# soldasim/BOSS.jl

Measured on AMD Instinct MI355X. Metric: gp_posterior_updates_per_sec (+ acq_evals_per_sec), N=4096 d=8 fp64, higher is better.
Workload: dtype f64; 1 GPU; d=8 synthetic blackbox, GaussianProcess(Matern52) surrogate, N=4096 fp64 posterior update + ExpectedImprovement over 8192 candidates per GPU (BASELINE.json configs[1]+[2]); N=4096, d=8, M_per_gpu=8192, kernel=matern52, parallelism=single GPU: no exchange

## Files before the change

### boss.jl_amd/csrc/chain.hpp

```cpp
#pragma once
#include "potrf.hpp"

namespace boss {

#ifdef BOSS_CHAIN_TRACE
__device__ unsigned long long g_ctrace[64 * 16];
#define CTRACE(step, slot) do { if ((threadIdx.x & 63) == 0) g_ctrace[((step) & 63) * 16 + (slot)] = __builtin_amdgcn_s_memrealtime(); } while (0)
#define CTRACE_MIN(step, slot) do { if (threadIdx.x == 0) atomicMin(&g_ctrace[((step) & 63) * 16 + (slot)], (unsigned long long)__builtin_amdgcn_s_memrealtime()); } while (0)
#define CTRACE_MAX(step, slot) do { if (threadIdx.x == 0) atomicMax(&g_ctrace[((step) & 63) * 16 + (slot)], (unsigned long long)__builtin_amdgcn_s_memrealtime()); } while (0)
#else
#define CTRACE(step, slot) do { } while (0)
#define CTRACE_MIN(step, slot) do { } while (0)
#define CTRACE_MAX(step, slot) do { } while (0)
#endif

#define CHAIN_CUT_VGPRS() asm volatile("" ::: "memory", "v0","v1","v2","v3","v4","v5","v6","v7","v8","v9","v10","v11","v12","v13","v14","v15","v16","v17","v18","v19","v20","v21","v22","v23","v24","v25","v26","v27","v28","v29","v30","v31","v32","v33","v34","v35","v36","v37","v38","v39","v40","v41","v42","v43","v44","v45","v46","v47","v48","v49","v50","v51","v52","v53","v54","v55","v56","v57","v58","v59","v60","v61","v62","v63","v64","v65","v66","v67","v68","v69","v70","v71","v72","v73","v74","v75","v76","v77","v78","v79","v80","v81","v82","v83","v84","v85","v86","v87","v88","v89","v90","v91","v92","v93","v94","v95","v96","v97","v98","v99","v100","v101","v102","v103","v104","v105","v106","v107","v108","v109","v110","v111")
constexpr int STRIPS_LDS_BYTES = 90 * 1024;
constexpr int CHAIN_CTRL = DIAG_TILES * 256 + DIAG_STAGE;
constexpr int CHAIN_LDS_BYTES = (CHAIN_CTRL + 2) * 8;


__device__ const unsigned char chain_tile_tab[16][3] = {
    {7, 0, 3}, {7, 3, 3}, {7, 6, 2}, {6, 0, 3}, {6, 3, 2}, {6, 5, 2}, {5, 0, 3}, {5, 3, 3},
    {4, 0, 3}, {4, 3, 2}, {3, 0, 2}, {3, 2, 2}, {2, 0, 3}, {1, 0, 2}, {0, 0, 1}, {0, 0, 0}};
__device__ __forceinline__ void chain_follow_phase(double* __restrict__ A, int ld, int b, int* __restrict__ info,
                                                             unsigned long long* __restrict__ sig, unsigned long long base, int wave_s,
                                                             unsigned budget) {
    extern __shared__ double smem[];
    int lane = (int)__builtin_amdgcn_mbcnt_hi(~0u, __builtin_amdgcn_mbcnt_lo(~0u, 0u));
    asm volatile("" : "+v"(lane));
    const int wave = wave_s, tid = wave * 64 + lane;
    const int r16 = lane & 15, q = lane >> 4;
    const int ti = chain_tile_tab[wave][0], tj0 = chain_tile_tab[wave][1], nt = chain_tile_tab[wave][2];
    constexpr int U = 3;
    const double* Ab = A + (size_t)b * BLK * ((size_t)ld + 1) + (size_t)q * ld + ti * 16 + r16;
    v4d cr[U];
#pragma unroll
    for (int u = 0; u < U; ++u) {
        const int tj = min(tj0 + u, ti);
#pragma unroll
        for (int i = 0; i < 4; ++i) cr[u][i] = ld_sc1(Ab + (size_t)(tj * 16 + 4 * i) * ld);
    }
    const unsigned long long pbase = base + 8ull * (b - 1);
    const double* Pl = A + (size_t)b * BLK + (size_t)(b - 1) * BLK * ld + (size_t)q * ld + r16;
    volatile lds_int_t* seenw = (volatile lds_int_t*)(unsigned)(unsigned long long)(smem + CHAIN_CTRL) + 1;
    auto poll_strips = [&]() {
        const unsigned long long v = lane < 8 ? ld_word(sig + SIGW_PROG + SIGW_PROG_STRIDE * lane) : ~0ull;
        const unsigned long long cnt = (v > pbase) ? v - pbase : 0ull;
        int mn = cnt > 8ull ? 8 : (int)cnt;
        mn = min(mn, __shfl_xor(mn, 1));
        mn = min(mn, __shfl_xor(mn, 2));
        mn = min(mn, __shfl_xor(mn, 4));
        return __builtin_amdgcn_readfirstlane(mn);
    };
    int seen = 0, jb = 0;
    bool dead = false;
    if (wave == 15) {
        if (lane == 0) CTRACE(b, 1);
        const PollTimer tm(budget);
        for (int it = 0; it < POLL_CAP && seen < 8; ++it) {
            const int mn = poll_strips();
            asm volatile("" ::: "memory");
            if (mn > seen) {
                seen = mn;
                if (lane == 0) *seenw = seen;
            }
            if (tm.check(it, info)) break;
            __builtin_amdgcn_s_sleep(1);
        }
        if (seen < 8) {
            if (lane == 0) {
                st_info(info, INT_MIN);
                note_giveup(4, b);
                *seenw = 99;
            }
        }
        if (lane == 0) CTRACE(b, 2);
        jb = 8;
    }
#pragma unroll 1
    while (jb < 8) {
        if (!dead && seen <= jb) {
            bool got = false;
            for (int it = 0; it < POLL_CAP_LDS; ++it) {
                const int v = *seenw;
                if (v > jb) {
                    seen = v;
                    got = v <= 8;
                    break;
                }
                __builtin_amdgcn_s_sleep(1);
            }
            if (!got) dead = true;
        }
        const bool two = (dead || seen >= jb + 2) && jb + 2 <= 8;
        const double* Pj = Pl + (size_t)(jb * 16) * ld;
        double bf[2][4], af[2][U][4];
#pragma unroll
        for (int s4 = 0; s4 < 4; ++s4) {
            bf[0][s4] = ld_sc1(Pj + (size_t)(4 * s4) * ld + ti * 16);
#pragma unroll
            for (int u = 0; u < U; ++u) af[0][u][s4] = ld_sc1(Pj + (size_t)(4 * s4) * ld + min(tj0 + u, ti) * 16);
        }
        if (two) {
#pragma unroll
            for (int s4 = 0; s4 < 4; ++s4) {
                bf[1][s4] = ld_sc1(Pj + (size_t)(16 + 4 * s4) * ld + ti * 16);
#pragma unroll
                for (int u = 0; u < U; ++u) af[1][u][s4] = ld_sc1(Pj + (size_t)(16 + 4 * s4) * ld + min(tj0 + u, ti) * 16);
            }
        }
#ifdef BOSS_CHAIN_TRACE
        if (wave == 0 && jb + (two ? 2 : 1) == 8) {
            asm volatile("s_waitcnt vmcnt(0)" ::: "memory");
            CTRACE(b, 11);
        }
#endif
#pragma unroll
        for (int s4 = 0; s4 < 4; ++s4)
#pragma unroll
            for (int u = 0; u < U; ++u) cr[u] = mfma_f64(-af[0][u][s4], bf[0][s4], cr[u]);
        if (two) {
#pragma unroll
            for (int s4 = 0; s4 < 4; ++s4)
#pragma unroll
                for (int u = 0; u < U; ++u) cr[u] = mfma_f64(-af[1][u][s4], bf[1][s4], cr[u]);
        }
        jb += two ? 2 : 1;
        if (!dead) {
            const int v = *seenw;
            if (v > seen && v <= 8) seen = v;
        }
    }
#pragma unroll
    for (int u = 0; u < U; ++u) {
        if (u < nt) {
            double* ct = smem + (ti * (ti + 1) / 2 + tj0 + u) * 256 + q * 16 + r16;
#pragma unroll
            for (int i = 0; i < 4; ++i) ct[64 * i] = cr[u][i];
        }
    }
    if (wave == 0) CTRACE(b, 12);
}

__device__ __forceinline__ void chain_factor_phase(double* __restrict__ Ab, int ld, double* __restrict__ inv16b, int col0,
                                                             unsigned long long* __restrict__ pubword, unsigned long long seq0,
                                                             int* __restrict__ info, int wave_s) {
    extern __shared__ double smem[];
    int fail = -1;
    int tid = wave_s * 64 + (int)__builtin_amdgcn_mbcnt_hi(~0u, __builtin_amdgcn_mbcnt_lo(~0u, 0u));
    asm volatile("" : "+v"(tid));
    diag_block_factor<false, false, true>(smem, Ab, ld, inv16b, col0, 8, fail, nullptr, pubword, seq0, info, tid + 0x10000);
}

__device__ __forceinline__ int chain_lane_opaque() {
    int lane = (int)__builtin_amdgcn_mbcnt_hi(~0u, __builtin_amdgcn_mbcnt_lo(~0u, 0u));
    asm volatile("" : "+v"(lane));
    return lane;
}

__global__ __launch_bounds__(DIAG_THREADS) void potrf_chain_kernel(double* __restrict__ A, int ld, int nblk,
                                                                   double* __restrict__ inv16, int* __restrict__ info,
                                                                   unsigned long long* __restrict__ sig, unsigned long long base,
                                                                   unsigned long long cbase, unsigned budget) {
    extern __shared__ double smem[];
    const int wave = __builtin_amdgcn_readfirstlane((int)threadIdx.x >> 6);
    volatile lds_int_t* ctrl = (volatile lds_int_t*)(unsigned)(unsigned long long)(smem + CHAIN_CTRL);
    asm volatile("" ::: "v127");
    if (threadIdx.x == 0) __hip_atomic_fetch_add(as_global(sig + SIGW_UP), 1ull, __ATOMIC_RELAXED, __HIP_MEMORY_SCOPE_AGENT);
    for (int b = blockIdx.x; b < nblk; b += gridDim.x) {
        double* Ab = A + (size_t)b * BLK * ((size_t)ld + 1);
        if (wave == 0) {
            const bool ok = b < 2 ? poll_ge(sig + SIGW_WDONE, base + 1, info, budget) : poll_ge(sig + SIGW_CRIT, cbase + 8ull * (b - 1), info, budget);
            if (chain_lane_opaque() == 0) {
                *ctrl = ok ? 1 : -1;
                ctrl[1] = 0;
            }
        }
        __syncthreads();
        if (*ctrl < 0) return;
        if (wave == 0) CTRACE(b, 0);
        __builtin_amdgcn_fence(__ATOMIC_ACQUIRE, "agent");
        if (b == 0) {
            const int lane = chain_lane_opaque();
            for (int tl = wave; tl < DIAG_TILES; tl += DIAG_THREADS / 64) {
                int ti = 0;
                while ((ti + 1) * (ti + 2) / 2 <= tl) ++ti;
                const int tj = tl - ti * (ti + 1) / 2;
#pragma unroll
                for (int h = 0; h < 2; ++h) {
                    const int e = lane + 64 * h, c = e >> 3, rp = e & 7;
                    *reinterpret_cast<v2d*>(smem + tl * 256 + c * 16 + 2 * rp) =
                        *reinterpret_cast<const v2d*>(Ab + (size_t)(tj * 16 + c) * ld + ti * 16 + 2 * rp);
                }
            }
        } else {
            CHAIN_CUT_VGPRS();
            chain_follow_phase(A, ld, b, info, sig, base, wave, budget);
        }
        CHAIN_CUT_VGPRS();
        __syncthreads();
        if (wave == 0) CTRACE(b, 3);
        chain_factor_phase(Ab, ld, inv16 + (size_t)b * (8 * 256), b * BLK, sig + SIGW_PANEL, base + 8ull * b, info, wave);
        CHAIN_CUT_VGPRS();
        if (wave == 15) CTRACE(b, 4);
        __syncthreads();
    }
}

template <bool CRIT>
__device__ __forceinline__ void follow_strip(double* __restrict__ A, int ld, int k, const double* __restrict__ inv16base,
                                             double* __restrict__ Brow, unsigned long long* __restrict__ prog,
                                             unsigned long long* __restrict__ sig, unsigned long long base, int* __restrict__ info,
                                             v4d (&xs)[TRSM_NA][64], int& ready, int& drained, int& avail, unsigned budget) {
    constexpr bool crit = CRIT;
    const int lane = threadIdx.x & 63;
    const int wave = __builtin_amdgcn_readfirstlane(threadIdx.x >> 6);
    const double* Lkk = A + (size_t)k * BLK * ((size_t)ld + 1);
    const double* inv16k = inv16base + (size_t)k * (8 * 256);
    const unsigned long long pb = base + 8ull * k;
    auto bload = [&](const double* p) { return crit ? ld_sc1(p) : *p; };
    auto panels_out = [&](unsigned long long v) { return v > pb ? (v - pb > 8ull ? 8 : (int)(v - pb)) : 0; };
    if (threadIdx.x == 0) {
        *(volatile lds_int_t*)&ready = 0;
        *(volatile lds_int_t*)&drained = 0;
        *(volatile lds_int_t*)&avail = panels_out(ld_word(sig + SIGW_PANEL));
    }
    __syncthreads();
    auto lval = [&](int jb, int m, int s) { return ld_sc1(Lkk + (size_t)(m * 16 + 4 * s + (lane >> 4)) * ld + jb * 16 + (lane & 15)); };
    auto ival = [&](int jb, int s) { return ld_sc1(inv16k + jb * 256 + (4 * s + (lane >> 4)) * 16 + (lane & 15)); };
    bool dead = false;
    auto ival_poll = [&](int jb, double (&iv)[4]) {
        const PollTimer tm(budget);
        for (int it = 0; it < POLL_CAP; ++it) {
            bool miss = false;
#pragma unroll
            for (int s = 0; s < 4; ++s) {
                iv[s] = ival(jb, s);
                miss |= __double_as_longlong(iv[s]) == -1ll;
            }
            if (!__any(miss)) return;
            if (dead) return;
            if (tm.check(it, info)) break;
            __builtin_amdgcn_s_sleep(1);
        }
        if (!dead && lane == 0) {
            st_info(info, INT_MIN);
            note_giveup(8, k);
        }
        dead = true;
        if (wave == 0 && lane == 0) *(volatile lds_int_t*)&avail = 99;
    };
    auto store_tile = [&](int jb, const v4d& t) {
#pragma unroll
        for (int i = 0; i < 4; ++i) {
            double* dst = Brow + (lane & 15) + (size_t)(jb * 16 + (lane >> 4) + 4 * i) * ld;
            if (crit) st_sc1(dst, t[i]);
            else *dst = t[i];
        }
    };
    int seen = *(volatile lds_int_t*)&avail;
    auto await = [&](int jb) {
        if (dead || seen > jb) return;
        if (wave == 0) {
            const PollTimer tm(budget);
            for (int i = 0; i < POLL_CAP; ++i) {
                seen = panels_out(ld_word(sig + SIGW_PANEL));
                if (seen > jb) {
                    asm volatile("" ::: "memory");
                    if (lane == 0) *(volatile lds_int_t*)&avail = seen;
                    return;
                }
                if (tm.check(i, info)) break;
                __builtin_amdgcn_s_sleep(crit ? 1 : 8);
            }
            dead = true;
            if (lane == 0) {
                st_info(info, INT_MIN);
                note_giveup(crit ? 5 : 6, k);
                *(volatile lds_int_t*)&avail = 99;
            }
        } else {
            for (int i = 0; i < POLL_CAP_LDS; ++i) {
                seen = *(volatile lds_int_t*)&avail;
                if (seen > jb) {
                    asm volatile("" ::: "memory");
                    if (seen > 8) dead = true;
                    return;
                }
                __builtin_amdgcn_s_sleep(2);
            }
            dead = true;
        }
    };
    const bool late = seen >= 8;
#ifdef BOSS_CHAIN_TRACE
    if (crit && blockIdx.x == 0 && threadIdx.x == 0) g_ctrace[(k & 63) * 16 + 7] = late ? 1 : 0;
    if (crit && blockIdx.x == 0 && threadIdx.x == 0) g_ctrace[(k & 63) * 16 + 8] = __builtin_amdgcn_s_memrealtime();
#endif
    if (wave == 0) {
        v4d acc[TRSM_NA];
#pragma unroll
        for (int jb = 0; jb < TRSM_NA; ++jb)
#pragma unroll
            for (int i = 0; i < 4; ++i) acc[jb][i] = bload(Brow + (lane & 15) + (size_t)(jb * 16 + (lane >> 4) + 4 * i) * ld);
        if (late) {
            double lv[TRSM_NA][TRSM_NA][4], iv[TRSM_NA][4];
#pragma unroll
            for (int jb = 0; jb < TRSM_NA; ++jb) {
#pragma unroll
                for (int s = 0; s < 4; ++s) iv[jb][s] = ival(jb, s);
#pragma unroll
                for (int m = 0; m < jb; ++m)
#pragma unroll
                    for (int s = 0; s < 4; ++s) lv[jb][m][s] = lval(jb, m, s);
            }
#pragma unroll
            for (int jb = 0; jb < TRSM_NA; ++jb) {
#pragma unroll
                for (int m = 0; m < jb; ++m)
#pragma unroll
                    for (int s = 0; s < 4; ++s) acc[jb] = mfma_f64(-lv[jb][m][s], acc[m][s], acc[jb]);
                v4d nw = {0.0, 0.0, 0.0, 0.0};
#pragma unroll
                for (int s = 0; s < 4; ++s) nw = mfma_f64(iv[jb][s], acc[jb][s], nw);
                acc[jb] = nw;
                xs[jb][lane] = nw;
                asm volatile("s_waitcnt lgkmcnt(0)" ::: "memory");
                if (lane == 0) *(volatile lds_int_t*)&ready = jb + 1;
            }
#pragma unroll
            for (int jb = 0; jb < TRSM_NA; ++jb) store_tile(jb, acc[jb]);
            if (crit) {
                drain_stores();
                if (lane == 0) raise_word(prog, pb + TRSM_NA);
            }
        } else {
#pragma unroll
            for (int jb = 0; jb < TRSM_NA; ++jb) {
                double iv[4], lv[TRSM_NA][4];
                if (crit) {
                    ival_poll(jb, iv);
                } else {
                    await(jb);
#pragma unroll
                    for (int s = 0; s < 4; ++s) iv[s] = ival(jb, s);
#pragma unroll
                    for (int j = jb + 1; j < TRSM_NA; ++j)
#pragma unroll
                        for (int s = 0; s < 4; ++s) lv[j][s] = lval(j, jb, s);
                }
                v4d nw = {0.0, 0.0, 0.0, 0.0};
#pragma unroll
                for (int s = 0; s < 4; ++s) nw = mfma_f64(iv[s], acc[jb][s], nw);
                acc[jb] = nw;
                xs[jb][lane] = nw;
                asm volatile("s_waitcnt lgkmcnt(0)" ::: "memory");
                if (lane == 0) *(volatile lds_int_t*)&ready = jb + 1;
                store_tile(jb, nw);
                if (crit) {
                    drain_stores();
                    if (lane == 0) raise_word(prog, pb + jb + 1);
                    await(jb);
#pragma unroll
                    for (int j = jb + 1; j < TRSM_NA; ++j)
#pragma unroll
                        for (int s = 0; s < 4; ++s) lv[j][s] = lval(j, jb, s);
                }
#pragma unroll
                for (int j = jb + 1; j < TRSM_NA; ++j)
#pragma unroll
                    for (int s = 0; s < 4; ++s) acc[j] = mfma_f64(-lv[j][s], nw[s], acc[j]);
            }
        }
        if (crit) {
            asm volatile("s_waitcnt vmcnt(0) lgkmcnt(0)" ::: "memory");
            if (lane == 0) *(volatile lds_int_t*)&drained = 1;
        }
#pragma unroll 1
        for (int jb = TRSM_NA; jb < 8; ++jb) await(jb);
    } else {
        constexpr int NB = 8 - TRSM_NA;
        v4d acc[NB];
#pragma unroll
        for (int j = 0; j < NB; ++j)
#pragma unroll
            for (int i = 0; i < 4; ++i) acc[j][i] = bload(Brow + (lane & 15) + (size_t)((TRSM_NA + j) * 16 + (lane >> 4) + 4 * i) * ld);
        auto hand_off = [&](int m) {
            while (*(volatile lds_int_t*)&ready <= m) __builtin_amdgcn_s_sleep(1);
            asm volatile("" ::: "memory");
            return xs[m][lane];
        };
        auto publish = [&](int upto) {
            if (!crit) return;
            drain_stores();
            while (*(volatile lds_int_t*)&drained == 0) __builtin_amdgcn_s_sleep(1);
            if (lane == 0) raise_word(prog, pb + upto);
        };
        if (late) {
            double lu[TRSM_NA][NB][4], lo[NB][NB][4], iv[NB][4];
#pragma unroll
            for (int m = 0; m < TRSM_NA; ++m)
#pragma unroll
                for (int j = 0; j < NB; ++j)
#pragma unroll
                    for (int s = 0; s < 4; ++s) lu[m][j][s] = lval(TRSM_NA + j, m, s);
#pragma unroll
            for (int j = 0; j < NB; ++j) {
#pragma unroll
                for (int s = 0; s < 4; ++s) iv[j][s] = ival(TRSM_NA + j, s);
#pragma unroll
                for (int m = 0; m < j; ++m)
#pragma unroll
                    for (int s = 0; s < 4; ++s) lo[j][m][s] = lval(TRSM_NA + j, TRSM_NA + m, s);
            }
#pragma unroll
            for (int m = 0; m < TRSM_NA; ++m) {
                const v4d x = hand_off(m);
#pragma unroll
                for (int s = 0; s < 4; ++s)
#pragma unroll
                    for (int j = 0; j < NB; ++j) acc[j] = mfma_f64(-lu[m][j][s], x[s], acc[j]);
            }
#pragma unroll
            for (int j = 0; j < NB; ++j) {
#pragma unroll
                for (int m = 0; m < j; ++m)
#pragma unroll
                    for (int s = 0; s < 4; ++s) acc[j] = mfma_f64(-lo[j][m][s], acc[m][s], acc[j]);
                v4d nw = {0.0, 0.0, 0.0, 0.0};
#pragma unroll
                for (int s = 0; s < 4; ++s) nw = mfma_f64(iv[j][s], acc[j][s], nw);
                acc[j] = nw;
            }
#pragma unroll
            for (int j = 0; j < NB; ++j) store_tile(TRSM_NA + j, acc[j]);
            publish(8);
        } else {
#pragma unroll
            for (int m = 0; m < TRSM_NA; ++m) {
                await(m);
                double lu[NB][4];
#pragma unroll
                for (int j = 0; j < NB; ++j)
#pragma unroll
                    for (int s = 0; s < 4; ++s) lu[j][s] = lval(TRSM_NA + j, m, s);
                const v4d x = hand_off(m);
#pragma unroll
                for (int s = 0; s < 4; ++s)
#pragma unroll
                    for (int j = 0; j < NB; ++j) acc[j] = mfma_f64(-lu[j][s], x[s], acc[j]);
            }
#pragma unroll
            for (int j = 0; j < NB; ++j) {
                double iv[4], lo[NB][4];
                if (crit) {
                    ival_poll(TRSM_NA + j, iv);
                } else {
                    await(TRSM_NA + j);
#pragma unroll
                    for (int s = 0; s < 4; ++s) iv[s] = ival(TRSM_NA + j, s);
#pragma unroll
                    for (int j2 = j + 1; j2 < NB; ++j2)
#pragma unroll
                        for (int s = 0; s < 4; ++s) lo[j2][s] = lval(TRSM_NA + j2, TRSM_NA + j, s);
                }
                v4d nw = {0.0, 0.0, 0.0, 0.0};
#pragma unroll
                for (int s = 0; s < 4; ++s) nw = mfma_f64(iv[s], acc[j][s], nw);
                acc[j] = nw;
                store_tile(TRSM_NA + j, nw);
                if (crit) {
                    publish(TRSM_NA + j + 1);
                    if (j + 1 < NB) {
                        await(TRSM_NA + j);
#pragma unroll
                        for (int j2 = j + 1; j2 < NB; ++j2)
#pragma unroll
                            for (int s = 0; s < 4; ++s) lo[j2][s] = lval(TRSM_NA + j2, TRSM_NA + j, s);
                    }
                }
#pragma unroll
                for (int j2 = j + 1; j2 < NB; ++j2)
#pragma unroll
                    for (int s = 0; s < 4; ++s) acc[j2] = mfma_f64(-lo[j2][s], nw[s], acc[j2]);
                if (!crit) publish(TRSM_NA + j + 1);
            }
        }
    }
}

__global__ __launch_bounds__(TRSM_THREADS) void potrf_follow_kernel(double* __restrict__ A, int ld, int k,
                                                                    const double* __restrict__ inv16base, int row0, int wait_rows,
                                                                    unsigned long long* __restrict__ sig, unsigned long long base,
                                                                    unsigned long long gateval, int* __restrict__ info, unsigned budget) {
    if (blockIdx.x == 0 && threadIdx.x == 0) {
        raise_word(sig + SIGW_WDONE, base + k + 1);
        if (gateval) raise_word(sig + SIGW_GATE, gateval);
    }
    __builtin_amdgcn_s_setprio(3);
    CTRACE_MIN(k, 5);
    __shared__ v4d xs[TRSM_NA][64];
// ... 70 lines not shown
```

### boss.jl_amd/csrc/potrf.hpp

```cpp
#pragma once
#include "gemm_f64.hpp"

namespace boss {

#ifdef BOSS_CHAIN_TRACE
__device__ unsigned long long g_cutrace[64 * 4];
__device__ unsigned long long g_ptrace[64 * 32];
#define PTRACE(col0, jb, slot) do { if ((threadIdx.x & 63) == 0) g_ptrace[(((col0) / BLK) & 63) * 32 + (slot) * 8 + (jb)] = __builtin_amdgcn_s_memrealtime(); } while (0)
#else
#define PTRACE(col0, jb, slot) do { } while (0)
#endif

__device__ __forceinline__ void lds_barrier() { asm volatile("s_waitcnt lgkmcnt(0)\n\ts_barrier" ::: "memory"); }


__device__ __forceinline__ void chol16_unscaled(v4d& S, v4d& E, double (&ipsel)[4], int lane, int col0, int& fail) {
    const int r16 = lane & 15, q = lane >> 4;
#pragma unroll
    for (int i = 0; i < 4; ++i) E[i] = (r16 == q + 4 * i) ? 1.0 : 0.0;
    bool bad = false;
    int badcol = 0;
#pragma unroll
    for (int t = 0; t < 4; ++t) {
        ipsel[t] = 1.0;
        double p = readlane_f64(S[t], 4 * t);
#pragma unroll
        for (int j = 0; j < 4; ++j) {
            double dn = 0.0, ln = 0.0, lS = 0.0, lE = 0.0, lc = 0.0;
            if (j < 3) {
                dn = readlane_f64(S[t], 16 * (j + 1) + 4 * t + j + 1);
                ln = readlane_f64(S[t], 16 * j + 4 * t + j + 1);
                lS = __shfl(S[t], 16 * j + r16);
                lE = __shfl(E[t], 16 * j + r16);
                lc = __shfl(S[t], 16 * j + 4 * t + q);
            }
            if (!(p > 0.0) && !bad) {
                bad = true;
                badcol = 4 * t + j;
            }
            const double ip = rcp_refined(p);
            ipsel[t] = (q == j) ? ip : ipsel[t];
            if (j < 3) {
                p = __builtin_fma(-ln, ln * ip, dn);
                const double lcm = (q > j) ? lc : 0.0;
                const double m = lcm * ip;
                S[t] = __builtin_fma(-lS, m, S[t]);
                E[t] = __builtin_fma(-lE, m, E[t]);
            }
        }
        if (t < 3) {
            const double am = (r16 > 4 * t + 3) ? -S[t] * ipsel[t] : 0.0;
            const double bS = S[t], bE = E[t];
            S = mfma_f64(am, bS, S);
            E = mfma_f64(am, bE, E);
        }
    }
    if (bad && fail < 0) fail = col0 + badcol;
}

__device__ __forceinline__ int lp_index(int R, int C) { return ((R * 4 + (C & 3)) * 4) + (C >> 2); }

typedef __attribute__((address_space(3))) int lds_int_t;
typedef __attribute__((address_space(1))) unsigned long long gmem_u64;
typedef __attribute__((address_space(1))) int gmem_i32;
__device__ __forceinline__ gmem_u64* as_global(const void* p) { return (gmem_u64*)(unsigned long long)p; }
__device__ __forceinline__ void st_sc1(double* p, double v) {
    __hip_atomic_store(as_global(p), (unsigned long long)__double_as_longlong(v), __ATOMIC_RELAXED, __HIP_MEMORY_SCOPE_AGENT);
}
__device__ __forceinline__ double ld_sc1(const double* p) {
    return __longlong_as_double((long long)__hip_atomic_load(as_global(p), __ATOMIC_RELAXED, __HIP_MEMORY_SCOPE_AGENT));
}
__device__ __forceinline__ unsigned long long ld_word(const unsigned long long* w) {
    return __hip_atomic_load(as_global(w), __ATOMIC_RELAXED, __HIP_MEMORY_SCOPE_AGENT);
}
__device__ __forceinline__ int ld_info(const int* p) {
    return __hip_atomic_load((gmem_i32*)(unsigned long long)p, __ATOMIC_RELAXED, __HIP_MEMORY_SCOPE_AGENT);
}
__device__ __forceinline__ void st_info(int* p, int v) {
    __hip_atomic_store((gmem_i32*)(unsigned long long)p, v, __ATOMIC_RELAXED, __HIP_MEMORY_SCOPE_AGENT);
}
__device__ __forceinline__ int ld_info_fresh(const int* p) {
    int r;
    const int zero = 0;
    asm volatile("global_atomic_or %0, %1, %2, off sc0\n\ts_waitcnt vmcnt(0)" : "=&v"(r) : "v"((gmem_i32*)(unsigned long long)p), "v"(zero) : "memory");
    return r;
}
__device__ __forceinline__ void st_sc1_x4(double* p, v2d v) {
    asm volatile("global_store_dwordx4 %0, %1, off sc1\n\ts_nop 1" ::"v"(as_global(p)), "v"(v) : "memory");
}
__device__ __forceinline__ void drain_stores() { asm volatile("s_waitcnt vmcnt(0)" ::: "memory"); }
__device__ __forceinline__ void raise_word(unsigned long long* w, unsigned long long v) {
    __hip_atomic_store(as_global(w), v, __ATOMIC_RELAXED, __HIP_MEMORY_SCOPE_AGENT);
}
constexpr int SIGW_GATE = 0, SIGW_BULK = 3, SIGW_PANEL = 16, SIGW_WDONE = 32, SIGW_CRIT = 48, SIGW_NEAR = 8, SIGW_PROG = 64, SIGW_PROG_STRIDE = 16,
              SIGW_UP = SIGW_PROG + 8 * SIGW_PROG_STRIDE,
              SIGW_DBG = SIGW_UP + 16,
              SIG_WORDS = SIGW_DBG + 16;
__device__ int g_giveup = 0;
#ifdef BOSS_DEBUG_WATCH_BUILD
__device__ unsigned long long* g_dbg = nullptr;
#endif
__device__ __forceinline__ void note_giveup(int code, int detail) {
    atomicCAS(&g_giveup, 0, code * 1000 + (detail & 511));
#ifdef BOSS_DEBUG_WATCH_BUILD
    unsigned long long* d = g_dbg;
    if (d) {
        atomicCAS(d + SIGW_DBG, 0ull, (unsigned long long)(code * 1000 + (detail & 511)));
        atomicAdd(d + SIGW_DBG + 1, 1ull);
        d[SIGW_DBG + 2] = (unsigned long long)(code * 1000 + (detail & 511));
    }
#endif
}
constexpr int POLL_CAP = 1 << 26;
constexpr int POLL_CAP_LDS = 1 << 22;
struct PollTimer {
    unsigned long long t0;
    unsigned budget;
    __device__ __forceinline__ explicit PollTimer(unsigned b) : t0(__builtin_amdgcn_s_memrealtime()), budget(b) {}
    __device__ __forceinline__ bool expired() const { return __builtin_amdgcn_s_memrealtime() - t0 > (unsigned long long)budget; }
    __device__ __forceinline__ int check(int i, const int* info) const {
        if ((i & 63) != 63) return 0;
        if (ld_info(info) == INT_MIN) return 2;
        if ((i & 1023) == 1023) {
            const int v = ld_info_fresh(info);
#ifdef BOSS_DEBUG_WATCH_BUILD
            if (v == INT_MIN && g_dbg && (threadIdx.x & 63) == 0) atomicAdd(g_dbg + SIGW_DBG + 4, 1ull);
#endif
            if (v == INT_MIN) return 2;
        }
        const bool out = expired();
#ifdef BOSS_DEBUG_WATCH_BUILD
        if (out && g_dbg && (threadIdx.x & 63) == 0) atomicAdd(g_dbg + SIGW_DBG + 5, 1ull);
#endif
        return out ? 1 : 0;
    }
};
__device__ __forceinline__ bool poll_ge(const unsigned long long* w, unsigned long long v, int* info, unsigned budget) {
    const PollTimer tm(budget);
    for (int i = 0; i < POLL_CAP; ++i) {
        if (ld_word(w) >= v) {
            asm volatile("" ::: "memory");
            return true;
        }
        const int st = tm.check(i, info);
        if (st == 2) return false;
        if (st == 1) break;
        __builtin_amdgcn_s_sleep(1);
    }
    if ((threadIdx.x & 63) == 0) {
        st_info(info, INT_MIN);
        note_giveup(1, (int)(v & 511));
    }
    return false;
}

constexpr int DIAG_THREADS = 1024;
constexpr int DIAG_TILES = 36;
constexpr int DIAG_STAGE = 2 * 256 + 2;
constexpr int DIAG_LDS_BYTES = (DIAG_TILES * 256 + DIAG_STAGE) * 8;
__device__ __forceinline__ int dtile(int i, int j) { return (i * (i + 1) / 2 + j) * 256; }
__device__ __forceinline__ double inv16_entry(double v) {
    const long long b = __double_as_longlong(v);
    return (b & 0x7fffffffffffffffll) > 0x7ff0000000000000ll ? __longlong_as_double(0x7ff8000000000000ll) : v;
}

template <bool KEEP = false, bool TILE0_GLOBAL = false, bool PUB = false>
__device__ __forceinline__ void diag_block_factor(double* __restrict__ smem, double* __restrict__ A, int ld,
                                                  double* __restrict__ inv16, int col0, int nsub, int& fail,
                                                  double* __restrict__ Is = nullptr, unsigned long long* pubword = nullptr,
                                                  unsigned long long pubseq0 = 0, int* info = nullptr, int tidtok = 0) {
    double* D = smem;
    double* Es = smem + DIAG_TILES * 256;
    double* Ss = Es + 256;
    volatile lds_int_t* xread = (volatile lds_int_t*)(unsigned)(unsigned long long)(Ss + 256);
    const int tid = tidtok >= 0x10000 ? tidtok - 0x10000 : (int)threadIdx.x + tidtok, lane = tid & 63;
    const int wave = __builtin_amdgcn_readfirstlane(tid >> 6);
    const int r16 = lane & 15, q = lane >> 4;
    constexpr int NW = DIAG_THREADS / 64;
    if (tid == 0) *xread = 0;
    v4d S = {0.0, 0.0, 0.0, 0.0};
    int osym[4], oel[4];
#pragma unroll
    for (int i = 0; i < 4; ++i) {
        const int c = q + 4 * i;
        osym[i] = (r16 >= c) ? (c * 16 + r16) : (r16 * 16 + c);
        oel[i] = c * 16 + r16;
    }
    int oe[4], od[4];
#pragma unroll
    for (int i = 0; i < 4; ++i) {
        oe[i] = lp_index(4 * i + q, r16);
        od[i] = lp_index(q + 4 * i, q + 4 * i);
    }
    const int olp = (r16 * 4 + q) * 4;
    if (wave == 0) {
#pragma unroll
        for (int i = 0; i < 4; ++i) {
            if constexpr (TILE0_GLOBAL) {
                const int c = q + 4 * i;
                S[i] = (r16 >= c) ? A[(size_t)c * ld + r16] : A[(size_t)r16 * ld + c];
            } else {
                S[i] = D[osym[i]];
            }
        }
    }
    for (int jb = 0; jb < nsub; ++jb) {
        const int t = nsub - 1 - jb;
        double ipsel[4];
        if (wave == 0) {
            v4d E;
            if constexpr (PUB) PTRACE(col0, jb, 0);
            chol16_unscaled(S, E, ipsel, lane, col0 + jb * 16, fail);
            if constexpr (PUB) PTRACE(col0, jb, 1);
            *reinterpret_cast<v4d*>(Es + olp) = E;
            *reinterpret_cast<v4d*>(Ss + olp) = S;
            if constexpr (PUB) {
                if (fail >= 0) {
                    if (lane == 0 && ld_info(info) == 0) st_info(info, fail + 1);
                    drain_stores();
                }
            }
        } else if (jb > 0 && (wave & 3) != 0 && !(PUB && wave == 15)) {
            const int jp = jb - 1, tp = nsub - 1 - jp;
            const int T = tp * (tp + 1) / 2;
            constexpr int U = 2;
            constexpr int NUPD = NW - NW / 4 - (PUB ? 1 : 0);
            const int uw = wave - 1 - (wave >> 2);
            for (int q0 = 1 + uw; q0 < T; q0 += U * NUPD) {
                int ti[U], tj[U];
                bool ok[U];
                v4d cr[U];
                double* ct[U];
#pragma unroll
                for (int u = 0; u < U; ++u) {
                    const int qq = q0 + NUPD * u;
                    ok[u] = qq < T;
                    int a = 0;
                    while ((a + 1) * (a + 2) / 2 <= qq) ++a;
                    const int b = qq - a * (a + 1) / 2;
                    ti[u] = ok[u] ? jp + 1 + a : jp + 2;
                    tj[u] = ok[u] ? jp + 1 + b : jp + 2;
                    ct[u] = D + dtile(ti[u], tj[u]);
#pragma unroll
                    for (int i = 0; i < 4; ++i) cr[u][i] = ct[u][oel[i]];
                }
#pragma unroll
                for (int s4 = 0; s4 < 4; ++s4) {
                    double af[U], bf[U];
#pragma unroll
                    for (int u = 0; u < U; ++u) {
                        af[u] = D[dtile(tj[u], jp) + oel[s4]];
                        bf[u] = D[dtile(ti[u], jp) + oel[s4]];
                    }
#pragma unroll
                    for (int u = 0; u < U; ++u) cr[u] = mfma_f64(-af[u], bf[u], cr[u]);
                }
#pragma unroll
                for (int u = 0; u < U; ++u) {
                    if (ok[u]) {
#pragma unroll
                        for (int i = 0; i < 4; ++i) ct[u][oel[i]] = cr[u][i];
                    }
                }
            }
        }
        lds_barrier();
        if (wave == 15) {
            const v4d Sv = *reinterpret_cast<const v4d*>(Ss + olp), Ev = *reinterpret_cast<const v4d*>(Es + olp);
            double* At = A + (size_t)(jb * 16) * ((size_t)ld + 1);
#pragma unroll
            for (int i = 0; i < 4; ++i) {
                const double rs = rsqrt_refined(Ss[od[i]]);
                const int c = q + 4 * i;
                if constexpr (PUB) {
                    if (r16 >= c) st_sc1(At + (size_t)c * ld + r16, Sv[i] * rs);
                    st_sc1(inv16 + jb * 256 + r16 * 16 + c, inv16_entry(Ev[i] * rs));
                } else {
                    if (r16 >= c) At[(size_t)c * ld + r16] = Sv[i] * rs;
                    inv16[jb * 256 + r16 * 16 + c] = inv16_entry(Ev[i] * rs);
                }
                if constexpr (KEEP) {
                    D[dtile(jb, jb) + oel[i]] = (r16 >= c) ? Sv[i] * rs : 0.0;
                    Is[jb * 256 + r16 * 16 + c] = Ev[i] * rs;
                }
            }
            if constexpr (PUB) {
                if (t == 0) {
                    drain_stores();
                    if (lane == 0) raise_word(pubword, pubseq0 + jb + 1);
                }
            }
        }
        if (t == 0) break;
        if (wave == 0) {
            const int tn = jb + 1;
            v4d P = {0.0, 0.0, 0.0, 0.0};
            const double* Dx = D + dtile(tn, jb);
            double aop[4], bop[4];
#pragma unroll
            for (int s4 = 0; s4 < 4; ++s4) {
                aop[s4] = Es[oe[s4]];
                bop[s4] = Dx[oel[s4]];
            }
            const double* Dn = D + dtile(tn, tn);
#pragma unroll
            for (int i = 0; i < 4; ++i) S[i] = Dn[osym[i]];
#pragma unroll
            for (int s4 = 0; s4 < 4; ++s4) P = mfma_f64(aop[s4], bop[s4], P);
            if (lane == 0) *xread = jb + 1;
#pragma unroll
            for (int s4 = 0; s4 < 4; ++s4) S = mfma_f64(-P[s4] * ipsel[s4], P[s4], S);
        } else if ((wave & 3) != 0 && wave - (wave >> 2) <= t) {
            const int wi = wave - (wave >> 2);
            const int tr = jb + wi;
            v4d P = {0.0, 0.0, 0.0, 0.0};
            double rs[4];
            double* Xt = D + dtile(tr, jb);
#pragma unroll
            for (int i = 0; i < 4; ++i) rs[i] = Ss[od[i]];
#pragma unroll
            for (int s4 = 0; s4 < 4; ++s4) {
                const double aop = Es[oe[s4]];
                const double bop = Xt[oel[s4]];
                P = mfma_f64(aop, bop, P);
            }
            double pv[4];
#pragma unroll
            for (int i = 0; i < 4; ++i) pv[i] = P[i] * rsqrt_refined(rs[i]);
            if (wi == 1) {
                while (*xread < jb + 1) __builtin_amdgcn_s_sleep(1);
            }
#pragma unroll
            for (int i = 0; i < 4; ++i) Xt[oel[i]] = pv[i];
        }
        lds_barrier();
        if constexpr (PUB) {
            if (wave == 15) {
                for (int tr = jb + 1; tr < nsub; ++tr) {
                    const double* src = D + dtile(tr, jb);
#pragma unroll
                    for (int h = 0; h < 2; ++h) {
                        const int e = lane + 64 * h, c = e >> 3, rp = e & 7;
                        st_sc1_x4(A + (size_t)(jb * 16 + c) * ld + tr * 16 + 2 * rp, *reinterpret_cast<const v2d*>(src + c * 16 + 2 * rp));
                    }
                }
                PTRACE(col0, jb, 2);
                drain_stores();
                PTRACE(col0, jb, 3);
                if (lane == 0) raise_word(pubword, pubseq0 + jb + 1);
            }
        }
        if constexpr (TILE0_GLOBAL) {
            if (wave == 12) {
                for (int tr = jb + 1; tr < nsub; ++tr) {
                    const double* src = D + dtile(tr, jb);
#pragma unroll
                    for (int h = 0; h < 2; ++h) {
                        const int e = lane + 64 * h, c = e >> 3, rp = e & 7;
                        *reinterpret_cast<v2d*>(A + (size_t)(jb * 16 + c) * ld + tr * 16 + 2 * rp) =
                            *reinterpret_cast<const v2d*>(src + c * 16 + 2 * rp);
                    }
                }
            }
        }
    }
}

__global__ __launch_bounds__(64) void potrf_gate_kernel(unsigned long long* __restrict__ sig, unsigned long long v,
                                                        int* __restrict__ info, unsigned budget) {
    if (threadIdx.x != 0) return;
    const PollTimer tm(budget);
    for (int i = 0; i < POLL_CAP; ++i) {
        if (__hip_atomic_load(sig, __ATOMIC_RELAXED, __HIP_MEMORY_SCOPE_AGENT) >= v) return;
        if ((i & 63) == 63 && tm.expired()) break;
        __builtin_amdgcn_s_sleep(16);
    }
    info[0] = INT_MIN;
    note_giveup(3, (int)(v & 511));
}

__global__ __launch_bounds__(64) void potrf_publish_kernel(unsigned long long* __restrict__ word, unsigned long long v) {
    if (threadIdx.x == 0) __hip_atomic_store(word, v, __ATOMIC_RELAXED, __HIP_MEMORY_SCOPE_AGENT);
}
__device__ __forceinline__ void wait_word(unsigned long long* w, unsigned long long v, int* info, unsigned budget) {
    if (!w) return;
    __shared__ int waited_s;
    if (threadIdx.x == 0) {
        bool ok = false, waited = false;
        const PollTimer tm(budget);
        for (int i = 0; i < POLL_CAP; ++i) {
            if (ld_word(w) >= v) {
                ok = true;
                break;
            }
            waited = true;
            if (tm.check(i, info)) break;
            __builtin_amdgcn_s_sleep(16);
        }
        if (!ok) {
            st_info(info, INT_MIN);
            note_giveup(2, (int)(v & 511));
        }
        *(volatile lds_int_t*)&waited_s = waited ? 1 : 0;
    }
    __syncthreads();
    if (*(volatile lds_int_t*)&waited_s) __builtin_amdgcn_fence(__ATOMIC_ACQUIRE, "agent");
}

__global__ __launch_bounds__(DIAG_THREADS) void potrf_diag_kernel(double* __restrict__ Abase, int ld, size_t bstride,
                                                                  int k, double* __restrict__ inv16base,
                                                                  size_t inv16_bstride, int* __restrict__ info,
                                                                  unsigned long long* sig, unsigned long long sigval) {
    extern __shared__ double smem[];
    const int tid = threadIdx.x;
    if (sig && tid == 0 && blockIdx.z == 0) __hip_atomic_store(sig, sigval, __ATOMIC_RELAXED, __HIP_MEMORY_SCOPE_AGENT);
    double* A = Abase + (size_t)blockIdx.z * bstride + (size_t)k * BLK * ((size_t)ld + 1);
    double* inv16 = inv16base + (size_t)blockIdx.z * inv16_bstride + (size_t)k * (8 * 256);
    const int lane = tid & 63, wv = tid >> 6;
    if (wv != 0) {
        for (int tl = wv; tl < DIAG_TILES; tl += DIAG_THREADS / 64 - 1) {
            int ti = 0;
            while ((ti + 1) * (ti + 2) / 2 <= tl) ++ti;
            const int tj = tl - ti * (ti + 1) / 2;
#pragma unroll
            for (int h = 0; h < 2; ++h) {
                const int e = lane + 64 * h, c = e >> 3, rp = e & 7;
                *reinterpret_cast<v2d*>(smem + tl * 256 + c * 16 + 2 * rp) =
                    *reinterpret_cast<const v2d*>(A + (size_t)(tj * 16 + c) * ld + ti * 16 + 2 * rp);
            }
        }
    }
    int fail = -1;
    diag_block_factor<false, true>(smem, A, ld, inv16, k * BLK, 8, fail);
    if (tid == 0 && fail >= 0) {
        if (info[blockIdx.z] == 0) info[blockIdx.z] = fail + 1;
    }
}

constexpr int SMALL_MAX_N = BLK, SMALL_MAX_D = 32;
struct SmallFitPar {
    int d, N, Np, ld, kern;
    double amp2, sig2;
    double invlam[SMALL_MAX_D];
};
constexpr int SMALL_LDS_DOUBLES = DIAG_TILES * 256 + DIAG_STAGE + 2 + 8 * 256 + SMALL_MAX_D * SMALL_MAX_N + 2 * SMALL_MAX_N + 8 + SMALL_MAX_D;
constexpr int SMALL_LDS_BYTES = SMALL_LDS_DOUBLES * 8;

__device__ __forceinline__ void small_fit_body(double* __restrict__ smem, int d, int N, int Np, int ld, int kern, double amp2,
                                               double sig2, const double* __restrict__ ilam, const double* __restrict__ Xraw,
                                               double* __restrict__ Xsc, const double* __restrict__ y,
                                               const double* __restrict__ mean, double* __restrict__ A,
                                               double* __restrict__ inv16, double* __restrict__ par_dev,
                                               double* __restrict__ scal, int* __restrict__ info,
                                               double* __restrict__ host_res, unsigned long long res_seq = 0) {
    double* Is = smem + DIAG_TILES * 256 + DIAG_STAGE + 2;
    double* xs = Is + 8 * 256;
    double* rhs = xs + SMALL_MAX_D * SMALL_MAX_N;
    double* red = rhs + 2 * SMALL_MAX_N;
    const int tid = threadIdx.x, lane = tid & 63, wv = tid >> 6;
    const int nsub = (N + 15) / 16;
    __syncthreads();
    if (par_dev) {
        if (tid < d) par_dev[tid] = ilam[tid];
        if (tid == 0) {
            par_dev[d] = amp2;
            par_dev[d + 1] = sig2;
        }
    }
    for (int idx = tid; idx < d * Np; idx += DIAG_THREADS) {
        const int k = idx / Np, j = idx - k * Np;
        const double v = Xraw[idx] * ilam[k];
        Xsc[idx] = v;
        if (j < SMALL_MAX_N) xs[k * SMALL_MAX_N + j] = v;
    }
    if (tid < SMALL_MAX_N) rhs[tid] = (tid < N) ? y[tid] - (mean ? mean[tid] : 0.0) : 0.0;
    __syncthreads();
    const int ntl = nsub * (nsub + 1) / 2;
    for (int idx = tid; idx < ntl * 256; idx += DIAG_THREADS) {
        const int tl = idx >> 8, e = idx & 255;
        int ti = 0;
        while ((ti + 1) * (ti + 2) / 2 <= tl) ++ti;
        const int tj = tl - ti * (ti + 1) / 2;
        const int r = e & 15, c = e >> 4, i = ti * 16 + r, j = tj * 16 + c;
        double v = 0.0;
        if (i >= j) {
            if (i < N && j < N) {
                double r2 = 0.0;
                for (int k = 0; k < d; ++k) {
                    const double diff = xs[k * SMALL_MAX_N + i] - xs[k * SMALL_MAX_N + j];
                    r2 = __builtin_fma(diff, diff, r2);
                }
                v = amp2 * kappa_r2(kern, r2) + ((i == j) ? sig2 : 0.0);
            } else {
                v = (i == j) ? 1.0 : 0.0;
            }
        }
        smem[tl * 256 + c * 16 + r] = v;
    }
    __syncthreads();
    int fail = -1;
    diag_block_factor<true>(smem, A, ld, inv16, 0, nsub, fail, Is);
    __syncthreads();
    if (wv == 0) {
        const int r16 = lane & 15, q = lane >> 4;
        double acc0 = 0.0, acc1 = 0.0;
        for (int jb = 0; jb < nsub; ++jb) {
            const int row0 = 16 * jb;
            if (lane >= (row0 & 63) && lane < (row0 & 63) + 16) rhs[row0 + (lane - (row0 & 63))] -= (row0 < 64) ? acc0 : acc1;
            double zs = 0.0;
#pragma unroll
            for (int i = 0; i < 4; ++i) {
                const int c = q + 4 * i;
                zs = __builtin_fma(Is[jb * 256 + c * 16 + r16], rhs[row0 + c], zs);
            }
            zs += __shfl_xor(zs, 16);
            zs += __shfl_xor(zs, 32);
            if (q == 0) rhs[SMALL_MAX_N + row0 + r16] = zs;
#pragma unroll
            for (int h = 0; h < 2; ++h) {
                const int row = lane + 64 * h, ti = row >> 4;
                if (ti > jb && ti < nsub) {
                    const double* Lt = smem + dtile(ti, jb) + (row & 15);
                    double a = 0.0;
#pragma unroll
                    for (int c = 0; c < 16; ++c) a = __builtin_fma(Lt[c * 16], rhs[SMALL_MAX_N + row0 + c], a);
                    if (h == 0) acc0 += a;
                    else acc1 += a;
                }
            }
        }
        double s0 = 0.0, s1 = 0.0;
#pragma unroll
        for (int h = 0; h < 2; ++h) {
            const int i = lane + 64 * h;
            if (i < N) {
                s0 += log(smem[dtile(i >> 4, i >> 4) + (i & 15) * 17]);
                const double z = rhs[SMALL_MAX_N + i];
                s1 = __builtin_fma(z, z, s1);
            }
        }
#pragma unroll
        for (int off = 32; off > 0; off >>= 1) {
            s0 += __shfl_xor(s0, off);
            s1 += __shfl_xor(s1, off);
        }
        if (lane == 0) {
            const int inf = fail >= 0 ? fail + 1 : 0;
            scal[0] = 2.0 * s0;
            scal[1] = s1;
            info[0] = inf;
            if (host_res) {
                host_res[0] = 2.0 * s0;
                host_res[1] = s1;
                reinterpret_cast<int*>(host_res + 2)[0] = inf;
                __threadfence_system();
                __hip_atomic_store(reinterpret_cast<unsigned long long*>(host_res + 3), res_seq, __ATOMIC_RELAXED, __HIP_MEMORY_SCOPE_SYSTEM);
            }
        }
    }
    __syncthreads();
    for (int tl = wv; tl < ntl; tl += DIAG_THREADS / 64) {
        int ti = 0;
        while ((ti + 1) * (ti + 2) / 2 <= tl) ++ti;
        const int tj = tl - ti * (ti + 1) / 2;
#pragma unroll
        for (int h = 0; h < 2; ++h) {
            const int e = lane + 64 * h, c = e >> 3, rp = e & 7;
            *reinterpret_cast<v2d*>(A + (size_t)(tj * 16 + c) * ld + ti * 16 + 2 * rp) =
                *reinterpret_cast<const v2d*>(smem + tl * 256 + c * 16 + 2 * rp);
        }
    }
    for (int c = tid; c < Np; c += DIAG_THREADS) {
        A[(size_t)c * ld + Np] = (c < 16 * nsub) ? rhs[SMALL_MAX_N + c] : 0.0;
        if (c >= 16 * nsub) A[(size_t)c * ld + c] = 1.0;
    }
    const int npan = Np / 16;
    for (int idx = tid; idx < (npan - nsub) * 256; idx += DIAG_THREADS) {
        const int pnl = nsub + (idx >> 8), e = idx & 255;
        inv16[pnl * 256 + e] = ((e & 15) == (e >> 4)) ? 1.0 : 0.0;
    }
}

__global__ __launch_bounds__(DIAG_THREADS) void small_fit_kernel(SmallFitPar par, const double* __restrict__ Xraw,
                                                                 double* __restrict__ Xsc, const double* __restrict__ y,
                                                                 const double* __restrict__ mean, double* __restrict__ A,
                                                                 double* __restrict__ inv16, double* __restrict__ par_dev,
                                                                 double* __restrict__ scal, int* __restrict__ info,
                                                                 double* __restrict__ host_res, unsigned long long res_seq) {
    extern __shared__ double smem[];
    double* ilam = smem + SMALL_LDS_DOUBLES - SMALL_MAX_D;
    if (threadIdx.x < par.d) ilam[threadIdx.x] = par.invlam[threadIdx.x];
    small_fit_body(smem, par.d, par.N, par.Np, par.ld, par.kern, par.amp2, par.sig2, ilam, Xraw, Xsc, y, mean, A, inv16, par_dev, scal,
                   info, host_res, res_seq);
}

__global__ __launch_bounds__(DIAG_THREADS) void small_fit_batch_kernel(int d, int N, int Np, int ld, int kern,
                                                                       const double* __restrict__ invlam,
                                                                       const double* __restrict__ hyp,
                                                                       const double* __restrict__ Xraw, double* __restrict__ Xsc,
                                                                       size_t sX, const double* __restrict__ y,
                                                                       const double* __restrict__ mean, size_t sMean,
                                                                       double* __restrict__ A, size_t sA, double* __restrict__ inv16,
                                                                       size_t sInv, double* __restrict__ scal, int* __restrict__ info) {
    extern __shared__ double smem[];
    const int b = blockIdx.x;
    double* ilam = smem + SMALL_LDS_DOUBLES - SMALL_MAX_D;
    if (threadIdx.x < d) ilam[threadIdx.x] = invlam[(size_t)b * d + threadIdx.x];
    small_fit_body(smem, d, N, Np, ld, kern, hyp[2 * b], hyp[2 * b + 1], ilam, Xraw, Xsc + (size_t)b * sX, y,
                   mean ? mean + (size_t)b * sMean : nullptr, A + (size_t)b * sA, inv16 + (size_t)b * sInv, nullptr, scal + 2 * b,
                   info + b, nullptr);
}

template <bool IDENTITY>
__device__ __forceinline__ void wave_trsm16(const double* __restrict__ Lkk, int ld,
                                            const double* __restrict__ inv16k, v4d (&acc)[8], int lane) {
#pragma unroll
    for (int jb = 0; jb < 8; ++jb) {
#pragma unroll
        for (int m = 0; m < jb; ++m) {
#pragma unroll
            for (int s = 0; s < 4; ++s) {
                double a = Lkk[(size_t)(m * 16 + 4 * s + (lane >> 4)) * ld + jb * 16 + (lane & 15)];
                acc[jb] = mfma_f64(-a, acc[m][s], acc[jb]);
            }
        }
        v4d nw = {0.0, 0.0, 0.0, 0.0};
#pragma unroll
        for (int s = 0; s < 4; ++s) {
            double a = inv16k[jb * 256 + (4 * s + (lane >> 4)) * 16 + (lane & 15)];
            nw = mfma_f64(a, acc[jb][s], nw);
        }
        acc[jb] = nw;
    }
}

constexpr int TRSM_NA = 5;
constexpr int TRSM_THREADS = 128;
__global__ __launch_bounds__(TRSM_THREADS) void potrf_trsm_kernel(double* __restrict__ Abase, int ld, size_t bstride, int k,
                                                                  const double* __restrict__ inv16base,
                                                                  size_t inv16_bstride, int row0) {
// ... 581 lines not shown
```

Measured before the change: 895.4 updates/s.

## Replace block barriers in published diag factor with per-tile LDS flag waits

In the PUB variant of diag_block_factor, the two block-wide lds_barrier calls per sub-column are replaced by fine-grained LDS progress words (staged, done-per-row, per-tile update counters). Waves poll only the specific tiles they depend on, so the diagonal Cholesky, TRSM and trailing-update waves can run out of lockstep. The LDS staging area is enlarged to hold the flag words, and these are reset by wave 15 before each panel. This adds polling overhead and ordering risk on LDS visibility, plus a give-up path that signals failure after a poll cap.

```diff
diff --git a/boss.jl_amd/csrc/chain.hpp b/boss.jl_amd/csrc/chain.hpp
--- a/boss.jl_amd/csrc/chain.hpp
+++ b/boss.jl_amd/csrc/chain.hpp
@@ -198,6 +198,7 @@
             CHAIN_CUT_VGPRS();
             chain_follow_phase(A, ld, b, info, sig, base, wave, budget);
         }
+        if (wave == 15) diag_words_reset(smem, chain_lane_opaque());
         CHAIN_CUT_VGPRS();
         __syncthreads();
         if (wave == 0) CTRACE(b, 3);
diff --git a/boss.jl_amd/csrc/potrf.hpp b/boss.jl_amd/csrc/potrf.hpp
--- a/boss.jl_amd/csrc/potrf.hpp
+++ b/boss.jl_amd/csrc/potrf.hpp
@@ -156,12 +156,50 @@
 
 constexpr int DIAG_THREADS = 1024;
 constexpr int DIAG_TILES = 36;
-constexpr int DIAG_STAGE = 2 * 256 + 2;
+constexpr int DIAG_STAGE = 2 * 256 + 32;
 constexpr int DIAG_LDS_BYTES = (DIAG_TILES * 256 + DIAG_STAGE) * 8;
 __device__ __forceinline__ int dtile(int i, int j) { return (i * (i + 1) / 2 + j) * 256; }
 __device__ __forceinline__ double inv16_entry(double v) {
     const long long b = __double_as_longlong(v);
     return (b & 0x7fffffffffffffffll) > 0x7ff0000000000000ll ? __longlong_as_double(0x7ff8000000000000ll) : v;
+}
+
+constexpr int DW_XREAD = 0,
+              DW_STAGED = 1,
+              DW_DONE = 8,
+              DW_UPD = 16,
+              DW_WORDS = 64;
+constexpr int POLL_CAP_PANEL = 1 << 20;
+#ifndef BOSS_DIAG_POLL_SLEEP
+#define BOSS_DIAG_POLL_SLEEP 1
+#endif
+template <int SLEEP>
+__device__ __forceinline__ void diag_wait_ge(volatile lds_int_t* w, int idx, bool need, int v, bool& dead, int* info, int lane) {
+    asm volatile("" ::: "memory");
+    if (dead) return;
+    for (int i = 0; i < POLL_CAP_PANEL; ++i) {
+        int x = v;
+        if (need) x = w[idx];
+        if (__all(x >= v)) {
+            asm volatile("" ::: "memory");
+            return;
+        }
+        if constexpr (SLEEP > 0) __builtin_amdgcn_s_sleep(SLEEP);
+    }
+    dead = true;
+    if (lane == 0 && info) {
+        st_info(info, INT_MIN);
+        note_giveup(12, v);
+    }
+}
+__device__ __forceinline__ void diag_raise(volatile lds_int_t* w, int idx, int v, bool who) {
+    asm volatile("" ::: "memory");
+    if (who) w[idx] = v;
+    asm volatile("" ::: "memory");
+}
+__device__ __forceinline__ void diag_words_reset(double* smem, int lane) {
+    volatile lds_int_t* w = (volatile lds_int_t*)(unsigned)(unsigned long long)(smem + DIAG_TILES * 256 + 2 * 256);
+    w[lane & (DW_WORDS - 1)] = 0;
 }
 
 template <bool KEEP = false, bool TILE0_GLOBAL = false, bool PUB = false>
@@ -177,7 +215,11 @@
     const int wave = __builtin_amdgcn_readfirstlane(tid >> 6);
     const int r16 = lane & 15, q = lane >> 4;
     constexpr int NW = DIAG_THREADS / 64;
-    if (tid == 0) *xread = 0;
+    if constexpr (!PUB) {
+        if (tid == 0) *xread = 0;
+    }
+    volatile lds_int_t* dw = xread;
+    bool dead = false;
     v4d S = {0.0, 0.0, 0.0, 0.0};
     int osym[4], oel[4];
 #pragma unroll
@@ -212,6 +254,9 @@
             if constexpr (PUB) PTRACE(col0, jb, 0);
             chol16_unscaled(S, E, ipsel, lane, col0 + jb * 16, fail);
             if constexpr (PUB) PTRACE(col0, jb, 1);
+            if constexpr (PUB) {
+                if (jb > 0) diag_wait_ge<0>(dw, DW_DONE + (lane & 7), lane <= nsub - jb, jb, dead, info, lane);
+            }
             *reinterpret_cast<v4d*>(Es + olp) = E;
             *reinterpret_cast<v4d*>(Ss + olp) = S;
             if constexpr (PUB) {
@@ -219,6 +264,7 @@
                     if (lane == 0 && ld_info(info) == 0) st_info(info, fail + 1);
                     drain_stores();
                 }
+                diag_raise(dw, DW_STAGED, jb + 1, lane == 0);
             }
         } else if (jb > 0 && (wave & 3) != 0 && !(PUB && wave == 15)) {
             const int jp = jb - 1, tp = nsub - 1 - jp;
@@ -226,6 +272,9 @@
             constexpr int U = 2;
             constexpr int NUPD = NW - NW / 4 - (PUB ? 1 : 0);
             const int uw = wave - 1 - (wave >> 2);
+            if constexpr (PUB) {
+                if (1 + uw < T) diag_wait_ge<BOSS_DIAG_POLL_SLEEP>(dw, DW_DONE + (lane & 7), lane >= 1 && lane <= tp, jb, dead, info, lane);
+            }
             for (int q0 = 1 + uw; q0 < T; q0 += U * NUPD) {
                 int ti[U], tj[U];
                 bool ok[U];
@@ -241,6 +290,14 @@
                     ti[u] = ok[u] ? jp + 1 + a : jp + 2;
                     tj[u] = ok[u] ? jp + 1 + b : jp + 2;
                     ct[u] = D + dtile(ti[u], tj[u]);
+                }
+                if constexpr (PUB) {
+                    static_assert(U == 2, "one lane per tile of the round");
+                    const int wix = DW_UPD + (lane == 0 ? dtile(ti[0], tj[0]) : dtile(ti[1], tj[1])) / 256;
+                    if (jp > 0) diag_wait_ge<BOSS_DIAG_POLL_SLEEP>(dw, wix, lane == 0 || (lane == 1 && ok[1]), jp, dead, info, lane);
+                }
+#pragma unroll
+                for (int u = 0; u < U; ++u) {
 #pragma unroll
                     for (int i = 0; i < 4; ++i) cr[u][i] = ct[u][oel[i]];
                 }
@@ -262,9 +319,17 @@
                         for (int i = 0; i < 4; ++i) ct[u][oel[i]] = cr[u][i];
                     }
                 }
-            }
-        }
-        lds_barrier();
+                if constexpr (PUB) {
+                    const int wix = DW_UPD + (lane == 0 ? dtile(ti[0], tj[0]) : dtile(ti[1], tj[1])) / 256;
+                    diag_raise(dw, wix, jb, lane == 0 || (lane == 1 && ok[1]));
+                }
+            }
+        }
+        if constexpr (PUB) {
+            if (wave == 15) diag_wait_ge<BOSS_DIAG_POLL_SLEEP>(dw, DW_STAGED, lane == 0, jb + 1, dead, info, lane);
+        } else {
+            lds_barrier();
+        }
         if (wave == 15) {
             const v4d Sv = *reinterpret_cast<const v4d*>(Ss + olp), Ev = *reinterpret_cast<const v4d*>(Es + olp);
             double* At = A + (size_t)(jb * 16) * ((size_t)ld + 1);
@@ -285,6 +350,7 @@
                 }
             }
             if constexpr (PUB) {
+                diag_raise(dw, DW_DONE, jb + 1, lane == 0);
                 if (t == 0) {
                     drain_stores();
                     if (lane == 0) raise_word(pubword, pubseq0 + jb + 1);
@@ -294,6 +360,9 @@
         if (t == 0) break;
         if (wave == 0) {
             const int tn = jb + 1;
+            if constexpr (PUB) {
+                if (jb > 0) diag_wait_ge<0>(dw, DW_UPD + dtile(tn, jb) / 256 + (lane & 1), lane < 2, jb, dead, info, lane);
+            }
             v4d P = {0.0, 0.0, 0.0, 0.0};
             const double* Dx = D + dtile(tn, jb);
             double aop[4], bop[4];
@@ -313,6 +382,10 @@
         } else if ((wave & 3) != 0 && wave - (wave >> 2) <= t) {
             const int wi = wave - (wave >> 2);
             const int tr = jb + wi;
+            if constexpr (PUB) {
+                diag_wait_ge<BOSS_DIAG_POLL_SLEEP>(dw, lane == 0 ? DW_STAGED : DW_UPD + dtile(tr, jb) / 256, lane == 0 || (lane == 1 && jb > 0),
+                                                   lane == 0 ? jb + 1 : jb, dead, info, lane);
+            }
             v4d P = {0.0, 0.0, 0.0, 0.0};
             double rs[4];
             double* Xt = D + dtile(tr, jb);
@@ -332,10 +405,12 @@
             }
 #pragma unroll
             for (int i = 0; i < 4; ++i) Xt[oel[i]] = pv[i];
-        }
-        lds_barrier();
+            if constexpr (PUB) diag_raise(dw, DW_DONE + wi, jb + 1, lane == 0);
+        }
+        if constexpr (!PUB) lds_barrier();
         if constexpr (PUB) {
             if (wave == 15) {
+                diag_wait_ge<BOSS_DIAG_POLL_SLEEP>(dw, DW_DONE + (lane & 7), lane >= 1 && lane <= t, jb + 1, dead, info, lane);
                 for (int tr = jb + 1; tr < nsub; ++tr) {
                     const double* src = D + dtile(tr, jb);
 #pragma unroll
```

New measurement: 874.9 updates/s. 2.3% lower.
